# patriciogonzalezvivo/prisma

Measured on AMD Instinct MI355X. Metric: frames/sec (depth_anything ViT-L + flow_raft, 1080p), higher is better.
Workload: dtype split-f16

## Files before the change

include/prisma_bands.h:

```cpp
#ifndef PRISMA_BANDS_H
#define PRISMA_BANDS_H

#include <stddef.h>
#include <stdint.h>

#ifdef __cplusplus
extern "C" {
#endif

typedef struct pb_ctx pb_ctx;

typedef enum {
    PB_OK = 0,
    PB_ERR_ARG = -1,
    PB_ERR_DEVICE = -2,
    PB_ERR_MEMORY = -3,
    PB_ERR_STATE = -4
} pb_status;

typedef enum { PB_F32 = 0, PB_F16 = 1, PB_U8 = 2, PB_I32 = 3 } pb_dtype;

typedef struct {
    const char *name;
    int32_t dtype;
// ... 254 lines not shown
                             void *bits, int inter_rows, float *inter);
int pb_op_mask_matrix_nms(pb_ctx *ctx, const float *inter, const float *area, const int *label, const float *score, int n, float sigma, int guard,
                          float *comp, float *out);
int pb_op_mask_sigmoid_rows(pb_ctx *ctx, const float *logit, int src_rows, int ld, const int *idx, int count, int HW, int guard_rows, float *sig);
int pb_op_mask_dynconv(pb_ctx *ctx, const float *kernels, int src_rows, const int *idx, int row_off, int M, const float *feat, int HW4, int split,
                       int guard_rows, float *out);
int pb_op_mask_band_accumulate(pb_ctx *ctx, const float *sig, const uint8_t *use, int k, int fh, int fw, int h, int w, int H, int W, float thr,
                               int guard, uint8_t *out, uint8_t *inst);
int pb_op_depth_layernorm(pb_ctx *ctx, const float *x, const float *g, const float *b, int B, int ntp, int ntok, int D, int drop_cls, int ldy, int lo_off,
                          int o8_off, float o8_scale, int lo8, int guard_rows, void *out, int *lo8_pa);
int pb_op_depth_attention(pb_ctx *ctx, const float *q, const float *k, const float *v, int B, int heads, int N, int variant, int ldo, int o8_off,
                          float o8_scale, int guard_rows, void *out);
int pb_op_depth_cls_rows(pb_ctx *ctx, const float *cls, const float *pos, int B, int ntp, int D, int guard_rows, float *out);
int pb_op_depth_dpt_tail(pb_ctx *ctx, const float *z, const float *bias, const float *w2, float b2, int B, int H, int W, int OH, int OW, int layout,
                         int ldz, int guard, float *out, int *lo8_pa);
int pb_op_depth_resize_minmax(pb_ctx *ctx, const float *net, int B, int nh, int nw, int H, int W, int guard, float *out, float *mnmx);
int pb_op_zoe_softplus(pb_ctx *ctx, float *x, int rows, int cols, int ld, int guard_rows);
int pb_op_zoe_dot32_relu(pb_ctx *ctx, const float *act, int ld, const float *w2, float b2, int rows, int guard, float *out);
int pb_op_zoe_bilerp_add(pb_ctx *ctx, const float *a, const float *src, int n, int h, int w, int H, int W, int C, int lda, int lds, int ldo,
                         int guard_rows, void *out);
int pb_op_zoe_attractor(pb_ctx *ctx, const float *A, int ldA, int nA, const float *bprev, int n, int h, int w, int H, int W, float alpha,
                        int guard_rows, float *out);
int pb_op_zoe_cat(pb_ctx *ctx, const float *act, int ld_act, const float *rel, const float *emb, int ld_emb, int n, int h, int w, int H, int W,
                  int guard_rows, void *out);
int pb_op_zoe_logbinom_depth(pb_ctx *ctx, const float *pt, int ld_pt, const float *bins, int n, int h, int w, int H, int W, float min_temp,
                             float max_temp, int guard, float *out);
int pb_op_zoe_pil_resize(pb_ctx *ctx, const float *in, int n, int h, int w, int H, int W, int guard, float *out);
int pb_op_bilinear(pb_ctx *ctx, const float *x, float *y, int B, int C, int H, int W, int OH, int OW,
                   int align_corners);
int pb_op_preprocess(pb_ctx *ctx, const uint8_t *frame, int H, int W, float *out, int net_h, int net_w);
// ... 8 lines not shown
```

prisma_amd/_lib.py:

```python
from __future__ import annotations

import ctypes as C
import os

_HERE = os.path.dirname(os.path.abspath(__file__))
LIB_PATH = os.environ.get("PRISMA_BANDS_LIB") or os.path.join(_HERE, "libprisma_bands.so")


class pb_tensor(C.Structure):
    _fields_ = [("name", C.c_char_p), ("dtype", C.c_int32), ("ndim", C.c_int32),
                ("shape", C.c_int64 * 6), ("data", C.c_void_p)]


class pb_depth_cfg(C.Structure):
    _fields_ = [("embed_dim", C.c_int32), ("depth", C.c_int32), ("heads", C.c_int32), ("features", C.c_int32),
                ("out_channels", C.c_int32 * 4), ("pos_grid", C.c_int32), ("max_batch", C.c_int32), ("metric", C.c_int32),
                ("precision", C.c_int32)]


class pb_flow_cfg(C.Structure):
    _fields_ = [("precision", C.c_int32)]


PREC_F16, PREC_SPLIT = 0, 1
# ... 144 lines not shown
    "pb_op_mask_coord_concat": (C.c_int, [_P, _P] + [C.c_int] * 7 + [_P]),
    "pb_op_mask_bilinear": (C.c_int, [_P, _P, _P] + [C.c_int] * 10 + [_P]),
    "pb_op_mask_gn_relu": (C.c_int, [_P, _P, _P, _P] + [C.c_int] * 5 + [_P, _P]),
    "pb_op_mask_cls_points_nms": (C.c_int, [_P, _P] + [C.c_int] * 6 + [_P]),
    "pb_op_mask_gather_rows": (C.c_int, [_P, _P, C.c_int, _P] + [C.c_int] * 5 + [_P]),
    "pb_op_mask_stats": (C.c_int, [_P, _P, C.c_int, C.c_int, C.c_int, C.c_float, C.c_int, _P]),
    "pb_op_mask_intersections": (C.c_int, [_P, _P, C.c_int, C.c_int, _P, C.c_int, C.c_int, C.c_float, C.c_int, _P, C.c_int, _P]),
    "pb_op_mask_matrix_nms": (C.c_int, [_P, _P, _P, _P, _P, C.c_int, C.c_float, C.c_int, _P, _P]),
    "pb_op_mask_sigmoid_rows": (C.c_int, [_P, _P, C.c_int, C.c_int, _P, C.c_int, C.c_int, C.c_int, _P]),
    "pb_op_mask_dynconv": (C.c_int, [_P, _P, C.c_int, _P, C.c_int, C.c_int, _P, C.c_int, C.c_int, C.c_int, _P]),
    "pb_op_mask_band_accumulate": (C.c_int, [_P, _P, _P] + [C.c_int] * 7 + [C.c_float, C.c_int, _P, _P]),
    "pb_op_depth_layernorm": (C.c_int, [_P, _P, _P, _P] + [C.c_int] * 8 + [C.c_float, C.c_int, C.c_int, _P, _P]),
    "pb_op_depth_attention": (C.c_int, [_P, _P, _P, _P] + [C.c_int] * 6 + [C.c_float, C.c_int, _P]),
    "pb_op_depth_cls_rows": (C.c_int, [_P, _P, _P] + [C.c_int] * 4 + [_P]),
    "pb_op_depth_dpt_tail": (C.c_int, [_P, _P, _P, _P, C.c_float] + [C.c_int] * 8 + [_P, _P]),
    "pb_op_depth_resize_minmax": (C.c_int, [_P, _P] + [C.c_int] * 6 + [_P, _P]),
    "pb_op_zoe_softplus": (C.c_int, [_P, _P] + [C.c_int] * 4),
    "pb_op_zoe_dot32_relu": (C.c_int, [_P, _P, C.c_int, _P, C.c_float, C.c_int, C.c_int, _P]),
    "pb_op_zoe_bilerp_add": (C.c_int, [_P, _P, _P] + [C.c_int] * 10 + [_P]),
    "pb_op_zoe_attractor": (C.c_int, [_P, _P, C.c_int, C.c_int, _P] + [C.c_int] * 5 + [C.c_float, C.c_int, _P]),
    "pb_op_zoe_cat": (C.c_int, [_P, _P, C.c_int, _P, _P] + [C.c_int] * 7 + [_P]),
    "pb_op_zoe_logbinom_depth": (C.c_int, [_P, _P, C.c_int, _P] + [C.c_int] * 5 + [C.c_float, C.c_float, C.c_int, _P]),
    "pb_op_zoe_pil_resize": (C.c_int, [_P, _P] + [C.c_int] * 6 + [_P]),
    "pb_op_bilinear": (C.c_int, [_P, _P, _P] + [C.c_int] * 7),
    "pb_op_preprocess": (C.c_int, [_P, _P, C.c_int, C.c_int, _P, C.c_int, C.c_int]),
    "pb_op_encode_depth": (C.c_int, [_P, _P, C.c_int, C.c_int, C.c_int, C.c_int, _P, _P, _P]),
}

_lib = None

# ... 33 lines not shown
```

prisma_amd/csrc/abi_ops.hip:

```cpp
#include <string.h>

#include <algorithm>
#include <vector>

#include "abi_ctx.h"
#include "corr_layout.h"
#include "gmflow_engine.h"
#include "mask_kernels.h"
#include "zoe_kernels.h"

namespace {
enum { SL_F16 = 0, SL_SPLIT16 = 1, SL_MX3 = 2, SL_MX2 = 3 };

class SplitOpEngine : public EngineBase {
  public:
    explicit SplitOpEngine(int device) : EngineBase(device) {}
    int setup(const pb_tensor *t, int n, int layout, int tapin) {
        PB_TRY(begin_load(t, n));
        split_w_ = layout != SL_F16; mx_ = layout >= SL_MX3; pack_mx2_ = layout == SL_MX2; pack_tapin_ = tapin;
        return 0;
    }
    int pack_layer(bool is_conv, int sa, int N, int K, PackedW &w) {
        if (is_conv) return pack_conv("l", true, nullptr, nullptr, w, sa);
        const pb_tensor *tw = find("l.weight"), *tb = find("l.bias");
// ... 831 lines not shown
    int dpt_tail(const float *z, const float *bias, const float *w2, float b2, int B, int H, int W, int OH, int OW, int layout, int ldz, int guard,
                 float *out) {
        const int Zp = 320, lo_off = layout ? Zp : 0;
        const int64_t P = (int64_t)B * H * W, px = (int64_t)B * OH * OW;
        std::vector<float> zp((size_t)P * Zp, 0.f);
        for (int64_t p = 0; p < P; ++p) memcpy(&zp[(size_t)p * Zp], z + p * 288, 288 * 4);
        std::vector<f16> hz((size_t)P * ldz);
        memset(hz.data(), 0xFF, hz.size() * 2);
        build_map(zp.data(), P, Zp, Zp, layout == 0 ? SL_F16 : (layout == 1 ? SL_SPLIT16 : SL_MX3), 1, ldz, hz);
        DevMem dz, dbias, dw2, dout;
        PB_TRY(up(dz, hz.data(), hz.size() * 2)); PB_TRY(up(dbias, bias, 32 * 4)); PB_TRY(up(dw2, w2, 32 * 4));
        PB_TRY(preset(dout, (size_t)(px + guard) * 4));
        PB_TRY(launch_dpt_tail(stream, dz.as<f16>(), B, H, W, ldz, lo_off, layout == 2 ? kLo8Pa : -1, dbias.as<float>(), dw2.as<float>(), b2, dout.as<float>(),
                               OH, OW));
        return finish(out, dout, (size_t)(px + guard) * 4);
    }

    int resize_minmax(const float *net, int B, int nh, int nw, int H, int W, int guard, float *out, float *mnmx) {
        const int64_t px = (int64_t)B * H * W;
        DevMem dn, dout, dmm;
        PB_TRY(up(dn, net, (size_t)B * nh * nw * 4));
        PB_TRY(preset(dout, (size_t)(px + guard) * 4));
        PB_TRY(dmm.alloc((size_t)B * 2 * 4));
        PB_TRY(launch_init_minmax(stream, dmm.as<unsigned>(), B));
        PB_TRY(launch_depth_resize_minmax(stream, dn.as<float>(), B, nh, nw, dout.as<float>(), H, W, dmm.as<unsigned>()));
        PB_TRY(finish(out, dout, (size_t)(px + guard) * 4));
        std::vector<unsigned> mm((size_t)B * 2);
        PB_TRY(down(mm.data(), dmm, mm.size() * 4));
        for (size_t i = 0; i < mm.size(); ++i) {
            const unsigned u = (mm[i] & 0x80000000u) ? (mm[i] & 0x7fffffffu) : ~mm[i];
// ... 1108 lines not shown
    return e.attention(q, k, v, B, heads, N, variant, ldo, o8_off, o8_scale, guard_rows, out);
}
int pb_op_depth_cls_rows(pb_ctx *c, const float *cls, const float *pos, int B, int ntp, int D, int guard_rows, float *out) {
    PB_CHECK(c && cls && pos && out && B > 0 && ntp > 0 && D > 0 && guard_rows >= 0, PB_ERR_ARG, "op_depth_cls_rows: bad arguments");
    DEPTH_OP_ENGINE(e);
    return e.cls_rows(cls, pos, B, ntp, D, guard_rows, out);
}
int pb_op_depth_dpt_tail(pb_ctx *c, const float *z, const float *bias, const float *w2, float b2, int B, int H, int W, int OH, int OW, int layout,
                         int ldz, int guard, float *out, int *lo8_pa) {
    PB_CHECK(c && z && bias && w2 && out && B > 0 && H > 0 && W > 0 && OH > 0 && OW > 0 && layout >= 0 && layout <= 2 && ldz % 8 == 0 &&
                 ldz >= (layout ? 640 : 320) && guard >= 0, PB_ERR_ARG, "op_depth_dpt_tail: bad arguments (a pixel is 320 halfs per part)");
    DEPTH_OP_ENGINE(e);
    if (lo8_pa) *lo8_pa = e.lo8_pa();
    return e.dpt_tail(z, bias, w2, b2, B, H, W, OH, OW, layout, ldz, guard, out);
}
int pb_op_depth_resize_minmax(pb_ctx *c, const float *net, int B, int nh, int nw, int H, int W, int guard, float *out, float *mnmx) {
    PB_CHECK(c && net && out && mnmx && B > 0 && nh > 0 && nw > 0 && H > 0 && W > 0 && guard >= 0, PB_ERR_ARG, "op_depth_resize_minmax: bad arguments");
    DEPTH_OP_ENGINE(e);
    return e.resize_minmax(net, B, nh, nw, H, W, guard, out, mnmx);
}
int pb_op_zoe_softplus(pb_ctx *c, float *x, int rows, int cols, int ld, int guard_rows) {
    PB_CHECK(c && x && rows > 0 && cols > 0 && ld >= cols && guard_rows >= 0, PB_ERR_ARG, "op_zoe_softplus: bad arguments");
    DEPTH_OP_ENGINE(e);
    return e.softplus(x, rows, cols, ld, guard_rows);
}
int pb_op_zoe_dot32_relu(pb_ctx *c, const float *act, int ld, const float *w2, float b2, int rows, int guard, float *out) {
    PB_CHECK(c && act && w2 && out && rows > 0 && ld >= 32 && ld % 8 == 0 && guard >= 0, PB_ERR_ARG, "op_zoe_dot32_relu: bad arguments");
    DEPTH_OP_ENGINE(e);
    return e.dot32_relu(act, ld, w2, b2, rows, guard, out);
}
// ... 35 lines not shown
```

prisma_amd/csrc/elementwise.hip:

```cpp
#include "kernels.h"

namespace {

__global__ __launch_bounds__(256) void layernorm_kernel(const float *__restrict__ x, const float *__restrict__ g,
                                                        const float *__restrict__ bt, f16 *__restrict__ y, int B,
                                                        int ntp, int ntok, int D, float eps, int drop_cls, int ldy,
                                                        int lo_off, int o8_off, float o8_scale, int lo8_pa) {
    const int lane = threadIdx.x & 63;
    const int64_t r = (int64_t)blockIdx.x * 4 + (threadIdx.x >> 6);
    if (r >= (int64_t)B * ntok) return;
    const int b = (int)(r / ntok), t = (int)(r - (int64_t)b * ntok);
    if (drop_cls && t == 0) return;
    const float *xr = x + ((int64_t)b * ntp + t) * D;
    f16 *yr = drop_cls ? y + ((int64_t)b * (ntok - 1) + (t - 1)) * ldy : y + ((int64_t)b * ntp + t) * ldy;
    f32x4 v[4];
    float s = 0.f;
#pragma unroll
    for (int j = 0; j < 4; ++j) {
        const int c = lane * 4 + 256 * j;
        if (c < D) {
            v[j] = *(const f32x4 *)(xr + c);
            s += (v[j][0] + v[j][1]) + (v[j][2] + v[j][3]);
        }
    }
// ... 689 lines not shown
    for (int j = 0; j < 8; ++j) s += fmaxf(acc[j] + bias[q4 * 8 + j], 0.f) * w2[q4 * 8 + j];
    s += __shfl_xor(s, 1);
    s += __shfl_xor(s, 2);
    if (live && q4 == 0) out[((int64_t)b * OH + Y) * OW + X] = fmaxf(s + b2, 0.f);
}

int launch_dpt_tail(hipStream_t s, const f16 *z, int B, int H, int W, int ldz, int lo_off, int lo8_pa, const float *bias, const float *w2, float b2,
                    float *out, int OH, int OW) {
    PB_CHECK(ldz % 8 == 0 && lo_off % 8 == 0 && (int64_t)H * W * ldz * 2 < (1LL << 31), -1, "dpt tail: pixel stride %d / residual offset %d must be multiples of 8, an image below 2 GB", ldz, lo_off);
    const float sy = bilerp_scale(H, OH, 1), sx = bilerp_scale(W, OW, 1);
    hipLaunchKernelGGL(dpt_tail_kernel, dim3((OW + 15) / 16, (OH + 3) / 4, B), dim3(256), 0, s, z, H, W, ldz, lo_off, lo8_pa, sy, sx, bias, w2, b2, out, OH, OW);
    PB_HIP(hipGetLastError());
    return 0;
}

int launch_bilinear_nhwc(hipStream_t s, const f16 *x, f16 *y, int B, int H, int W, int OH, int OW, int C, int ldc,
                         int align, int lo_off, int lo8_pa) {
    PB_CHECK(C % 8 == 0 && ldc % 8 == 0, -1, "bilinear: C=%d ldc=%d must be multiples of 8", C, ldc);
    const float sy = bilerp_scale(H, OH, align), sx = bilerp_scale(W, OW, align);
    hipLaunchKernelGGL(bilinear_nhwc_kernel, dim3(nblk((int64_t)B * OH * OW * (C / 8))), dim3(256), 0, s, x, y, B, H,
                       W, OH, OW, C / 8, ldc, align, sy, sx, lo_off, lo8_pa);
    PB_HIP(hipGetLastError());
    return 0;
}

int launch_init_minmax(hipStream_t s, unsigned *mm, int B) {
    hipLaunchKernelGGL(init_minmax_kernel, dim3(nblk(B)), dim3(256), 0, s, mm, B);
    PB_HIP(hipGetLastError());
    return 0;
}
// ... 95 lines not shown
```

prisma_amd/csrc/engine.h:

```cpp
#pragma once
#include <map>
#include <string>
#include <vector>

#include "engine_base.h"
#include "zoe_kernels.h"

class DepthEngine : public EngineBase {
  public:
    DepthEngine(int device, const pb_depth_cfg &cfg, const CreateEnv &env = create_env());
    int load(const pb_tensor *w, int n);
    int infer(const uint8_t *frames_dev, int n, int H, int W, float *depth_out, uint8_t *rgb_out, float *mn,
              float *mx, int flip);
    int max_batch() const { return cfg_.max_batch > 0 ? cfg_.max_batch : 1; }

  private:
    int prepare(int B, int H, int W);
    int run_chunk(const uint8_t *frames, int n, float *depth_out, uint8_t *rgb_out, float *mn, float *mx, int flip);
    int vit(int n);
    int head(int f0, int n);
    int tail(int n, float *depth_out, uint8_t *rgb_out, float *mn, float *mx, int flip);
    int load_metric();
    int plan_metric(int B, int H, int W);
    int metric_tables(int H, int W);
// ... 9 lines not shown
    int head_tapin_ = 1;
    int vit_sw_ = 0, head_sa_ = 0, head_sw_ = 0, hs_ = 1;
    int vit_res_ = 15;
    int vit_mx_ = 0, head_mx_ = 0;
    int batch_cap(int H, int W) const;
    PackedW patch_;
    float *cls_ = nullptr;
    std::vector<float> pos_host_;
    struct Block { float *ln1g, *ln1b, *ln2g, *ln2b, *ls1, *ls2; PackedW qkv, proj, fc1, fc2; };
    std::vector<Block> blocks_;
    float *normg_ = nullptr, *normb_ = nullptr;
    PackedW proj_[4], rs0_, rs1_, rs3_, rn_[4], outc_[4], rcu_[4][2][2], oc1_, oc2_;
    PackedW wz_;
    int head_tail_ = 1;
    f16 *z_ = nullptr;
    float *w2_ = nullptr;
    float b2_ = 0.f;
    static constexpr int64_t kSkFloats = (int64_t)512 * 128 * 128;

    int pB_ = 0, pH_ = 0, pW_ = 0;
    int hB_ = 1;
    int nh_ = 0, nw_ = 0, gh_ = 0, gw_ = 0, ntok_ = 0, ntp_ = 0, P_ = 0;
    int lh_[4] = {0, 0, 0, 0}, lw_[4] = {0, 0, 0, 0};
    int *xi_ = nullptr, *yi_ = nullptr;
    float *xw_ = nullptr, *yw_ = nullptr, *pos_ = nullptr;
    f16 *patchA_ = nullptr, *Y_ = nullptr, *Q_ = nullptr, *K_ = nullptr, *Vt_ = nullptr, *AO_ = nullptr, *Hd_ = nullptr;
    float *X_ = nullptr;
    f16 *feat_[4] = {nullptr, nullptr, nullptr, nullptr};
    f16 *pj_[4] = {}, *lay_[4] = {}, *rnraw_[4] = {}, *rnrelu_[4] = {}, *tmp_[4] = {}, *sraw_[4] = {}, *srelu_[4] = {},
        *yb_[4] = {}, *ocb_[4] = {}, *path_[4] = {};
// ... 13 lines not shown
```

prisma_amd/csrc/engine.hip:

```cpp
#include "engine.h"

#include <math.h>
#include <stdlib.h>
#include <string.h>

#include <algorithm>

namespace {
const char *const kFam[] = {"gemm_f16", "conv_igemm_f16", "attention", "layernorm", "elementwise", "prepost", "gemm_f16_resid",
                            "gemm_f16_qkv"};
enum { F_GEMM_RESID = 6, F_GEMM_QKV = 7 };
inline int cp64(int c) { return (int)round_up(c, 64); }
}

DepthEngine::DepthEngine(int dev, const pb_depth_cfg &cfg, const CreateEnv &env) : EngineBase(dev, env, kFam), cfg_(cfg) {}

PackSpec DepthEngine::spec(int sa, int sw, int mx2) const {
    PackSpec s;
    s.sa = sa; s.sw = sw; s.mx = head_mx_; s.mx2 = mx2; s.tapin = head_tapin_;
    return s;
}

int DepthEngine::pack_vit(const float *wt, int N, int K, PackedW &out, const float *bias, bool keep_res) {
    if (vit_mx_) return pack_spec(wt, N, K, K, out, bias, 1, keep_res ? spec(0, 1, 1) : spec(0, 0));
// ... 101 lines not shown
        if ((r = pack_conv(Hh + "projects." + std::to_string(i), oc[i], D, 1, true, proj_[i]))) return r;
        if ((r = pack_conv(Hh + "scratch.layer" + std::to_string(i + 1) + "_rn", F, oc[i], 3, false, rn_[i]))) return r;
        const std::string rf = Hh + "scratch.refinenet" + std::to_string(i + 1) + ".";
        if ((r = pack_conv(rf + "out_conv", F, F, 1, true, outc_[i]))) return r;
        for (int u = 0; u < 2; ++u)
            for (int c = 0; c < 2; ++c)
                if ((r = pack_conv(rf + "resConfUnit" + std::to_string(u + 1) + ".conv" + std::to_string(c + 1), F, F, 3,
                                   true, rcu_[i][u][c])))
                    return r;
    }
    if ((r = pack_convT(Hh + "resize_layers.0", oc[0], 4, rs0_))) return r;
    if ((r = pack_convT(Hh + "resize_layers.1", oc[1], 2, rs1_))) return r;
    if ((r = pack_conv(Hh + "resize_layers.3", oc[3], oc[3], 3, true, rs3_))) return r;
    if ((r = pack_conv(Hh + "scratch.output_conv1", F / 2, F, 3, true, oc1_))) return r;
    if ((r = pack_conv(Hh + "scratch.output_conv2.0", 32, F / 2, 3, true, oc2_))) return r;
    head_tail_ = env.head_tail && !cfg_.metric;
    if (head_tail_) {
        const int ci = F / 2, cip = cp64(ci);
        const float *wt = need(Hh + "scratch.output_conv2.0.weight", (int64_t)32 * ci * 9);
        if (!wt) return PB_ERR_ARG;
        std::vector<float> g((size_t)288 * cip, 0.f);
        for (int c = 0; c < 32; ++c)
            for (int k = 0; k < ci; ++k)
                for (int t = 0; t < 9; ++t) g[((size_t)t * 32 + c) * cip + k] = wt[((size_t)c * ci + k) * 9 + t];
        if ((r = pack_spec(g.data(), 288, cip, cip, wz_, nullptr, 1, spec(head_sa_, head_sw_)))) return r;
        wz_.Kreal = ci;
    }
    UP(w2_, Hh + "scratch.output_conv2.2.weight", 32);
    { NEED(b2, Hh + "scratch.output_conv2.2.bias", 1); b2_ = b2[0]; }
#undef NEED
#undef UP
    if (cfg_.metric) {
        int rm = load_metric();
        if (rm) return rm;
    }
    tmap_.clear();
    PB_HIP(hipDeviceSynchronize());
    return 0;
}

namespace {
// ... 129 lines not shown
        const size_t mxs = vit_mx_ ? 3 : 2;
        Y_ = (f16 *)carve((size_t)rows * D * mxs);
        const size_t qkb = (size_t)B * cfg_.heads * ntp_ * 64 * 2 + slack;
        Q_ = (f16 *)carve(qkb); K_ = (f16 *)carve(qkb); Vt_ = (f16 *)carve(qkb);
        AO_ = (f16 *)carve((size_t)rows * D * mxs);
        Hd_ = (f16 *)carve((size_t)rows * 4 * D * mxs);
        for (int i = 0; i < 4; ++i) feat_[i] = (f16 *)carve((size_t)round_up((int64_t)B * P_, 256) * D * 2 * hs_);
        for (int i = 0; i < 4; ++i) {
            const size_t pix = (size_t)round_up((int64_t)HB * lh_[i] * lw_[i], 256) * hs_;
            const int ocp = cp64(cfg_.out_channels[i]);
            pj_[i] = (f16 *)carve((size_t)round_up((int64_t)HB * P_, 256) * ocp * 2 * hs_);
            lay_[i] = i == 2 ? pj_[2] : (f16 *)carve(pix * ocp * 2);
            rnraw_[i] = (f16 *)carve(pix * Fp * 2); rnrelu_[i] = (f16 *)carve(pix * Fp * 2);
            tmp_[i] = (f16 *)carve(pix * Fp * 2);
            sraw_[i] = (f16 *)carve(pix * Fp * 2); srelu_[i] = (f16 *)carve(pix * Fp * 2);
            yb_[i] = (f16 *)carve(pix * Fp * 2); ocb_[i] = (f16 *)carve(pix * Fp * 2);
            const int th = i == 0 ? 2 * lh_[0] : lh_[i - 1], tw = i == 0 ? 2 * lw_[0] : lw_[i - 1];
            path_[i] = (f16 *)carve((size_t)round_up((int64_t)HB * th * tw, 256) * Fp * 2 * hs_);
        }
        o1_ = (f16 *)carve((size_t)round_up((int64_t)HB * 4 * lh_[0] * lw_[0], 256) * F2p * 2 * hs_);
        if (head_tail_) z_ = (f16 *)carve((size_t)round_up((int64_t)HB * 4 * lh_[0] * lw_[0], 256) * cp64(288) * 2 * hs_);
        else up_ = (f16 *)carve((size_t)round_up((int64_t)HB * nh_ * nw_, 256) * F2p * 2 * hs_);
        netd_ = (float *)carve((size_t)HB * nh_ * nw_ * 4);
        full_ = (float *)carve((size_t)HB * H * W * 4);
        mm_ = (unsigned *)carve((size_t)HB * 8);
        return cfg_.metric ? plan_metric(HB, H, W) : 0;
    });
    if (r) return r;
    std::vector<int> xi, yi;
    std::vector<float> xw, yw, pos;
    if (cfg_.metric) {
// ... 142 lines not shown
        if ((r = conv3(lay_[i], cp64(oc[i]), n, lh_[i], lw_[i], rn_[i], rnraw_[i], rnrelu_[i], nullptr, nullptr, ACT_NONE,
                       1, Fp)))
            return r;
        nhwc("layer" + std::to_string(i + 1) + "_rn", rnraw_[i], F, lh_[i], lw_[i], Fp);
    }
    for (int lv = 3; lv >= 0; --lv) {
        const int h = lh_[lv], w = lw_[lv];
        const f16 *sr = rnraw_[lv], *sl = rnrelu_[lv];
        if (lv < 3) {
            if ((r = conv3(rnrelu_[lv], Fp, n, h, w, rcu_[lv][0][0], tmp_[lv], nullptr, nullptr, nullptr, ACT_RELU, 1, Fp))) return r;
            if ((r = conv3(tmp_[lv], Fp, n, h, w, rcu_[lv][0][1], sraw_[lv], srelu_[lv], rnraw_[lv], path_[lv + 1], ACT_NONE, 1, Fp))) return r;
            sr = sraw_[lv]; sl = srelu_[lv];
        }
        if ((r = conv3(sl, Fp, n, h, w, rcu_[lv][1][0], tmp_[lv], nullptr, nullptr, nullptr, ACT_RELU, 1, Fp))) return r;
        if ((r = conv3(tmp_[lv], Fp, n, h, w, rcu_[lv][1][1], yb_[lv], nullptr, sr, nullptr, ACT_NONE, 1, Fp))) return r;
        {
            GemmArgs a;
            a.A = yb_[lv]; a.lda = hs * Fp; a.M = n * h * w; a.out = ocb_[lv]; a.ldo = hs * Fp; a.lo_off = lo(Fp);
            if ((r = gemm(A_DENSE, EPI_STD, a, outc_[lv]))) return r;
        }
        const int th = lv == 0 ? 2 * h : lh_[lv - 1], tw = lv == 0 ? 2 * w : lw_[lv - 1];
        if ((r = bil(ocb_[lv], path_[lv], h, w, th, tw, F, Fp))) return r;
        nhwc("path" + std::to_string(lv + 1), path_[lv], F, th, tw, Fp);
    }
    const int h1 = 2 * lh_[0], w1 = 2 * lw_[0];
    if ((r = conv3(path_[0], Fp, n, h1, w1, oc1_, o1_, nullptr, nullptr, nullptr, ACT_NONE, 1, F2p))) return r;
    nhwc("output_conv1", o1_, F2, h1, w1, F2p);
    if (head_tail_) {
        const int Zp = cp64(288);
        GemmArgs a;
        a.A = o1_; a.lda = hs * F2p; a.M = n * h1 * w1; a.out = z_; a.ldo = hs * Zp; a.lo_off = lo(Zp); a.N = 288;
        if ((r = gemm(A_DENSE, EPI_STD, a, wz_))) return r;
        r = timed(F_ELT, 0, (double)n * ((double)h1 * w1 * 288 * (head_sa_ ? 3.0 : 2.0) + (double)nh_ * nw_ * 4.0), [&] {
            return launch_dpt_tail(stream, z_, n, h1, w1, hs * Zp, lo(Zp), head_mx_ ? kLo8Pa : -1, oc2_.bias, w2_, b2_, netd_, nh_, nw_);
        });
        if (r) return r;
        stages_["net_depth"] = Stage::f32_rows(netd_, n, nh_, nw_);
        return 0;
    }
    if ((r = bil(o1_, up_, h1, w1, nh_, nw_, F2, F2p))) return r;
    if (cfg_.metric) {
// ... 84 lines not shown
```

prisma_amd/csrc/kernels.h:

```cpp
#pragma once
#include "common.h"

int launch_attention(hipStream_t s, const f16 *q, const f16 *k, const f16 *vt, f16 *o, int B, int heads, int ntp,
                     int ntok, int ldo, int variant = 0, int o8_off = 0, float o8_scale = 16.f);

int launch_layernorm(hipStream_t s, const float *x, const float *g, const float *b, f16 *y, int B, int ntp, int ntok,
                     int D, float eps, int drop_cls, int ldy = 0, int lo_off = 0, int o8_off = 0, float o8_scale = 16.f, int lo8_pa = -1);

int launch_cls_rows(hipStream_t s, float *resid, const float *cls, const float *pos, int B, int ntp, int D);

int launch_preprocess(hipStream_t s, const uint8_t *frames, int B, int H, int W, int nh, int nw, const int *xi,
                      const float *xw, const int *yi, const float *yw, f16 *out, int Kp, float *chw_out);

int launch_bilinear_nhwc(hipStream_t s, const f16 *x, f16 *y, int B, int H, int W, int OH, int OW, int C, int ldc,
                         int align_corners, int lo_off = 0, int lo8_pa = -1);

int launch_dpt_tail(hipStream_t s, const f16 *z, int B, int H, int W, int ldz, int lo_off, int lo8_pa, const float *bias, const float *w2, float b2,
                    float *out, int OH, int OW);

int launch_depth_resize_minmax(hipStream_t s, const float *net, int B, int nh, int nw, float *out, int H, int W,
                               unsigned *mm);
int launch_minmax_only(hipStream_t s, const float *x, int B, int64_t per, unsigned *mm);
int launch_heat_encode(hipStream_t s, const float *depth, int B, int H, int W, const unsigned *mm, int flip,
                       uint8_t *rgb, float *mn, float *mx);
int launch_init_minmax(hipStream_t s, unsigned *mm, int B);
int launch_still_encode(hipStream_t s, const float *depth, int H, int W, unsigned *mm, unsigned *g2max, uint8_t *q, int flip, int encode_range,
                        uint8_t *rgb, float *mnmx);
int launch_point_cloud(hipStream_t s, const float *depth, const uint8_t *rgb, int n, int H, int W, int flip, float u0, float v0, float fx,
                       float fy, unsigned *mm, uint8_t *out);
int launch_hue_heat(hipStream_t s, const uint8_t *frames, int n, int H, int W, int y0, int x0, int Hd, int Wd, uint8_t *depth_out, float *heat_out);

int launch_nchw_f32_to_nhwc_f16(hipStream_t s, const float *x, f16 *y, int B, int C, int H, int W, int ldc, int relu);
int launch_nhwc_f16_to_nchw_f32(hipStream_t s, const f16 *x, float *y, int B, int C, int H, int W, int ldc);
// ... 16 lines not shown
```

prisma_amd/engine.py:

```python
from __future__ import annotations

import ctypes as C
from typing import Dict, List, Optional, Tuple

import numpy as np

from . import _lib
from ._lib import check
from .synth import DEPTH_CFGS, MASK_CFGS, DepthCfg, MaskCfg


def _ptr(a: Optional[np.ndarray]):
    return None if a is None else a.ctypes.data_as(C.c_void_p)


def _f32(a) -> np.ndarray:
    return np.ascontiguousarray(a, dtype=np.float32)


VERTEX_DTYPE = np.dtype([("x", "<f4"), ("y", "<f4"), ("z", "<f4"), ("red", "u1"), ("green", "u1"), ("blue", "u1")])


def device_count() -> int:
    return _lib.load().pb_device_count()
# ... 966 lines not shown
    def depth_cls_rows(self, cls, pos, B: int, ntp: int, guard_rows: int = 2) -> np.ndarray:
        cls, pos = _f32(cls), _f32(pos)
        out = np.empty((B * ntp + guard_rows, cls.shape[0]), np.float32)
        check(self.lib.pb_op_depth_cls_rows(self.ctx, _ptr(cls), _ptr(pos), B, ntp, cls.shape[0], guard_rows, _ptr(out)))
        return out

    def depth_dpt_tail(self, z, bias, w2, b2: float, OH: int, OW: int, layout: int, ldz: int, guard: int = 64):
        z, bias, w2 = _f32(z), _f32(bias), _f32(w2)
        B, H, W, Cc = z.shape
        assert Cc == 288 and bias.shape == (32,) and w2.shape == (32,)
        out = np.empty(B * OH * OW + guard, np.float32)
        pa = C.c_int(-1)
        check(self.lib.pb_op_depth_dpt_tail(self.ctx, _ptr(z), _ptr(bias), _ptr(w2), b2, B, H, W, OH, OW, layout, ldz, guard, _ptr(out), C.byref(pa)))
        return out, pa.value

    def depth_resize_minmax(self, net, H: int, W: int, guard: int = 64):
        net = _f32(net)
        B, nh, nw = net.shape
        out = np.empty(B * H * W + guard, np.float32)
        mm = np.empty((B, 2), np.float32)
        check(self.lib.pb_op_depth_resize_minmax(self.ctx, _ptr(net), B, nh, nw, H, W, guard, _ptr(out), _ptr(mm)))
        return out, mm

    def zoe_softplus(self, buf, rows: int, cols: int) -> np.ndarray:
        buf = _f32(buf).copy()
        check(self.lib.pb_op_zoe_softplus(self.ctx, _ptr(buf), rows, cols, buf.shape[1], buf.shape[0] - rows))
        return buf

    def zoe_dot32_relu(self, act, ld: int, w2, b2: float, guard: int = 8) -> np.ndarray:
        act, w2 = _f32(act), _f32(w2)
# ... 351 lines not shown
```

Before: 138.0.

## Fold refinenet1 out_conv into output_conv1 and run conv after upsample as gather

The refinenet1 1x1 out_conv weights are composed with the 3x3 output_conv1 weights on the host at setup. One GEMM now runs at low resolution and produces 9 taps times F/2 channels. A new gather kernel then bilinearly upsamples those per-tap partial sums and adds them at the 2x resolution. This replaces the path of 1x1 conv, bilinear upsample to a full-width buffer, then a 3x3 conv at high resolution, so high-resolution FLOPs and traffic drop. The cost is a wider intermediate (9*F/2 channels) and composed weights whose rounding differs slightly. It is on by default unless the head_tail env bit 2 is set.

```diff
diff --git a/include/prisma_bands.h b/include/prisma_bands.h
--- a/include/prisma_bands.h
+++ b/include/prisma_bands.h
@@ -292,6 +292,8 @@
 int pb_op_depth_cls_rows(pb_ctx *ctx, const float *cls, const float *pos, int B, int ntp, int D, int guard_rows, float *out);
 int pb_op_depth_dpt_tail(pb_ctx *ctx, const float *z, const float *bias, const float *w2, float b2, int B, int H, int W, int OH, int OW, int layout,
                          int ldz, int guard, float *out, int *lo8_pa);
+int pb_op_depth_oc1(pb_ctx *ctx, const float *x, const float *wo, const float *bo, const float *w1, const float *b1, int B, int H, int W, int F, int layout,
+                    int route, int guard_rows, void *out, int *lo8_pa);
 int pb_op_depth_resize_minmax(pb_ctx *ctx, const float *net, int B, int nh, int nw, int H, int W, int guard, float *out, float *mnmx);
 int pb_op_zoe_softplus(pb_ctx *ctx, float *x, int rows, int cols, int ld, int guard_rows);
 int pb_op_zoe_dot32_relu(pb_ctx *ctx, const float *act, int ld, const float *w2, float b2, int rows, int guard, float *out);
diff --git a/prisma_amd/_lib.py b/prisma_amd/_lib.py
--- a/prisma_amd/_lib.py
+++ b/prisma_amd/_lib.py
@@ -182,6 +182,7 @@
     "pb_op_depth_attention": (C.c_int, [_P, _P, _P, _P] + [C.c_int] * 6 + [C.c_float, C.c_int, _P]),
     "pb_op_depth_cls_rows": (C.c_int, [_P, _P, _P] + [C.c_int] * 4 + [_P]),
     "pb_op_depth_dpt_tail": (C.c_int, [_P, _P, _P, _P, C.c_float] + [C.c_int] * 8 + [_P, _P]),
+    "pb_op_depth_oc1": (C.c_int, [_P] * 6 + [C.c_int] * 7 + [_P, _P]),
     "pb_op_depth_resize_minmax": (C.c_int, [_P, _P] + [C.c_int] * 6 + [_P, _P]),
     "pb_op_zoe_softplus": (C.c_int, [_P, _P] + [C.c_int] * 4),
     "pb_op_zoe_dot32_relu": (C.c_int, [_P, _P, C.c_int, _P, C.c_float, C.c_int, C.c_int, _P]),
diff --git a/prisma_amd/csrc/abi_ops.hip b/prisma_amd/csrc/abi_ops.hip
--- a/prisma_amd/csrc/abi_ops.hip
+++ b/prisma_amd/csrc/abi_ops.hip
@@ -6,6 +6,7 @@
 #include "abi_ctx.h"
 #include "corr_layout.h"
 #include "gmflow_engine.h"
+#include "head_linear.h"
 #include "mask_kernels.h"
 #include "zoe_kernels.h"
 
@@ -869,6 +870,37 @@
         PB_TRY(launch_dpt_tail(stream, dz.as<f16>(), B, H, W, ldz, lo_off, layout == 2 ? kLo8Pa : -1, dbias.as<float>(), dw2.as<float>(), b2, dout.as<float>(),
                                OH, OW));
         return finish(out, dout, (size_t)(px + guard) * 4);
+    }
+
+    int oc1(const float *x, const float *wo, const float *bo, const float *w1, const float *b1, int B, int H, int W, int F, int layout, int route, int guard,
+            void *out) {
+        const int F2 = F / 2, F2p = (int)round_up(F2, 64), sa = layout != SL_F16, hs = sa ? 2 : 1, Zp = (int)round_up(9 * F2, 64);
+        const int64_t P = (int64_t)B * H * W, OP = 4 * P, ldo = hs * F2p;
+        const int lo8 = layout == SL_MX3 ? kLo8Pa : -1;
+        std::vector<f16> hx((size_t)round_up(P, 256) * hs * F, (f16)0.f);
+        build_map(x, P, F, F, layout, sa, hs * F, hx);
+        DevMem dx, db1, dout, dz, dp;
+        PB_TRY(up(dx, hx.data(), hx.size() * 2)); PB_TRY(up(db1, b1, (size_t)F2 * 4));
+        PB_TRY(preset(dout, (size_t)(round_up(OP, 256) + guard) * ldo * 2));
+        if (route) {
+            std::vector<double> g, gb;
+            pb_compose_oc1(w1, wo, bo, F, F, g, gb);
+            const std::vector<float> gf(g.begin(), g.end()), gbf(gb.begin(), gb.end());
+            PackedW wz;
+            PB_TRY(pack(gf.data(), 9 * F2, F, F, wz, gbf.data(), 1, sa));
+            PB_TRY(preset(dz, (size_t)round_up(P, 256) * hs * Zp * 2));
+            PB_TRY(dense(dx.as<f16>(), hs * F, P, wz, dz.as<f16>(), hs * Zp, ACT_NONE, nullptr, 0, -1, sa ? Zp : 0));
+            PB_TRY(launch_dpt_oc1_gather(stream, dz.as<f16>(), B, H, W, F2, hs * Zp, sa ? Zp : 0, lo8, db1.as<float>(), dout.as<f16>(), (int)ldo, sa ? F2p : 0));
+        } else {
+            PackedW wc, w3;
+            PB_TRY(pack(wo, F, F, F, wc, bo, 1, sa));
+            PB_TRY(pack(pb_conv_rows(w1, F2, F, 9, F).data(), F2, 9 * F, 9 * F, w3, b1, 9, sa));
+            PB_TRY(preset(dz, (size_t)round_up(P, 256) * hs * F * 2)); PB_TRY(preset(dp, (size_t)round_up(OP, 256) * hs * F * 2));
+            PB_TRY(dense(dx.as<f16>(), hs * F, P, wc, dz.as<f16>(), hs * F, ACT_NONE, nullptr, 0, -1, sa ? F : 0));
+            PB_TRY(launch_bilinear_nhwc(stream, dz.as<f16>(), dp.as<f16>(), B, H, W, 2 * H, 2 * W, F, hs * F, 1, sa ? F : 0, lo8));
+            PB_TRY(conv(dp.as<f16>(), F, 0, B, 2 * H, 2 * W, 3, 3, 1, w3, dout.as<f16>(), (int)ldo, ACT_NONE, 0, nullptr, nullptr, sa ? F2p : 0));
+        }
+        return finish(out, dout, (size_t)(OP + guard) * ldo * 2);
     }
 
     int resize_minmax(const float *net, int B, int nh, int nw, int H, int W, int guard, float *out, float *mnmx) {
@@ -2007,6 +2039,16 @@
     if (lo8_pa) *lo8_pa = e.lo8_pa();
     return e.dpt_tail(z, bias, w2, b2, B, H, W, OH, OW, layout, ldz, guard, out);
 }
+int pb_op_depth_oc1(pb_ctx *c, const float *x, const float *wo, const float *bo, const float *w1, const float *b1, int B, int H, int W, int F, int layout,
+                    int route, int guard_rows, void *out, int *lo8_pa) {
+    PB_CHECK(c && x && wo && bo && w1 && b1 && out && B > 0 && H > 0 && W > 0 && F > 0 && F % 64 == 0 && layout >= SL_F16 && layout <= SL_MX3 &&
+                 (route == 0 || route == 1) && guard_rows >= 0, PB_ERR_ARG, "op_depth_oc1: bad arguments (F a multiple of 64; layout 0 f16, 1 split16, 2 mx3)");
+    PB_HIP(hipSetDevice(c->device));
+    DepthOpEngine e(c->device);
+    PB_TRY(e.setup(nullptr, 0, layout, 1));
+    if (lo8_pa) *lo8_pa = e.lo8_pa();
+    return e.oc1(x, wo, bo, w1, b1, B, H, W, F, layout, route, guard_rows, out);
+}
 int pb_op_depth_resize_minmax(pb_ctx *c, const float *net, int B, int nh, int nw, int H, int W, int guard, float *out, float *mnmx) {
     PB_CHECK(c && net && out && mnmx && B > 0 && nh > 0 && nw > 0 && H > 0 && W > 0 && guard >= 0, PB_ERR_ARG, "op_depth_resize_minmax: bad arguments");
     DEPTH_OP_ENGINE(e);
diff --git a/prisma_amd/csrc/elementwise.hip b/prisma_amd/csrc/elementwise.hip
--- a/prisma_amd/csrc/elementwise.hip
+++ b/prisma_amd/csrc/elementwise.hip
@@ -727,6 +727,117 @@
     return 0;
 }
 
+__global__ __launch_bounds__(256) void dpt_oc1_gather_kernel(const f16 *__restrict__ z, int H, int W, int C, int ldz, int lo_off, int lo8_pa, float sy, float sx,
+                                                             const float *__restrict__ bias, f16 *__restrict__ out, int ldo, int olo_off, int OH, int OW,
+                                                             int TW, int TH) {
+    const int C8 = C >> 3, cg = threadIdx.x % C8, p = threadIdx.x / C8;
+    const int X = blockIdx.x * TW + p % TW, Y = blockIdx.y * TH + p / TW, b = blockIdx.z;
+    if (p >= TW * TH || X >= OW || Y >= OH) return;
+    int y0[3], y1[3], x0[3], x1[3];
+    float ly[3], lx[3];
+    bool oky[3], okx[3];
+#pragma unroll
+    for (int t = 0; t < 3; ++t) {
+        const int qy = Y + t - 1, qx = X + t - 1;
+        oky[t] = qy >= 0 && qy < OH; okx[t] = qx >= 0 && qx < OW;
+        bilerp_src(oky[t] ? qy : 0, sy, H, 1, y0[t], y1[t], ly[t]);
+        bilerp_src(okx[t] ? qx : 0, sx, W, 1, x0[t], x1[t], lx[t]);
+    }
+    const __amdgpu_buffer_rsrc_t rs = make_rsrc(z + (int64_t)b * H * W * ldz, (unsigned)((int64_t)H * W * ldz * 2));
+    const int lane_ch = cg * 8;
+    typedef int i32x4v __attribute__((ext_vector_type(4)));
+    typedef int i32x2v __attribute__((ext_vector_type(2)));
+    const float inv = __builtin_ldexpf(1.f, -(lo8_pa + 12));
+    float acc[8];
+#pragma unroll
+    for (int j = 0; j < 8; ++j) acc[j] = 0.f;
+#pragma unroll
+    for (int ky = 0; ky < 3; ++ky)
+#pragma unroll
+        for (int kx = 0; kx < 3; ++kx) {
+            if (!(oky[ky] && okx[kx])) continue;
+            const int ch = (ky * 3 + kx) * C + lane_ch;
+            const int o[4] = {(y0[ky] * W + x0[kx]) * ldz, (y0[ky] * W + x1[kx]) * ldz, (y1[ky] * W + x0[kx]) * ldz, (y1[ky] * W + x1[kx]) * ldz};
+            const float hy = 1.f - ly[ky], hx = 1.f - lx[kx];
+            const float w4[4] = {hy * hx, hy * lx[kx], ly[ky] * hx, ly[ky] * lx[kx]};
+            f16x8 h[4];
+#pragma unroll
+            for (int n = 0; n < 4; ++n) h[n] = __builtin_bit_cast(f16x8, (i32x4v)__builtin_amdgcn_raw_buffer_load_b128(rs, (o[n] + ch) * 2, 0, 0));
+            if (lo_off && lo8_pa >= 0) {
+                int2 u[4];
+#pragma unroll
+                for (int n = 0; n < 4; ++n) {
+                    const i32x2v t2 = (i32x2v)__builtin_amdgcn_raw_buffer_load_b64(rs, o[n] * 2 + 3 * lo_off + ch, 0, 0);
+                    u[n].x = t2[0]; u[n].y = t2[1];
+                }
+#pragma unroll
+                for (int n = 0; n < 4; ++n) {
+                    const float wl = w4[n] * inv;
+#pragma unroll
+                    for (int j = 0; j < 8; ++j) acc[j] += w4[n] * (float)h[n][j];
+#pragma unroll
+                    for (int hh = 0; hh < 2; ++hh) {
+                        const int wv = hh ? u[n].y : u[n].x;
+                        const f32x2 a = __builtin_amdgcn_cvt_pk_f32_fp8(wv, false), d = __builtin_amdgcn_cvt_pk_f32_fp8(wv, true);
+                        acc[4 * hh + 0] += wl * a[0]; acc[4 * hh + 1] += wl * a[1]; acc[4 * hh + 2] += wl * d[0]; acc[4 * hh + 3] += wl * d[1];
+                    }
+                }
+            } else if (lo_off) {
+#pragma unroll
+                for (int n = 0; n < 4; ++n) {
+                    const f16x8 l = __builtin_bit_cast(f16x8, (i32x4v)__builtin_amdgcn_raw_buffer_load_b128(rs, (o[n] + ch + lo_off) * 2, 0, 0));
+#pragma unroll
+                    for (int j = 0; j < 8; ++j) acc[j] += w4[n] * ((float)h[n][j] + (float)l[j]);
+                }
+            } else {
+#pragma unroll
+                for (int n = 0; n < 4; ++n)
+#pragma unroll
+                    for (int j = 0; j < 8; ++j) acc[j] += w4[n] * (float)h[n][j];
+            }
+        }
+    const float4 b0 = *(const float4 *)(bias + lane_ch), b1 = *(const float4 *)(bias + lane_ch + 4);
+    const float bs[8] = {b0.x, b0.y, b0.z, b0.w, b1.x, b1.y, b1.z, b1.w};
+    f16 *dst = out + (((int64_t)b * OH + Y) * OW + X) * ldo + lane_ch;
+    f16x8 o;
+#pragma unroll
+    for (int j = 0; j < 8; ++j) {
+        acc[j] += bs[j];
+        o[j] = (f16)acc[j];
+    }
+    *(f16x8 *)dst = o;
+    if (olo_off && lo8_pa >= 0) {
+        const float shi = __builtin_ldexpf(1.f, lo8_pa), slo = __builtin_ldexpf(1.f, lo8_pa + 12);
+        int2 h8, l8;
+        h8.x = pb_fp8x4((float)o[0] * shi, (float)o[1] * shi, (float)o[2] * shi, (float)o[3] * shi);
+        h8.y = pb_fp8x4((float)o[4] * shi, (float)o[5] * shi, (float)o[6] * shi, (float)o[7] * shi);
+        l8.x = pb_fp8x4((acc[0] - (float)o[0]) * slo, (acc[1] - (float)o[1]) * slo, (acc[2] - (float)o[2]) * slo, (acc[3] - (float)o[3]) * slo);
+        l8.y = pb_fp8x4((acc[4] - (float)o[4]) * slo, (acc[5] - (float)o[5]) * slo, (acc[6] - (float)o[6]) * slo, (acc[7] - (float)o[7]) * slo);
+        char *d8 = (char *)(dst - lane_ch) + lane_ch;
+        *(int2 *)(d8 + 2 * olo_off) = h8;
+        *(int2 *)(d8 + 3 * olo_off) = l8;
+    } else if (olo_off) {
+        f16x8 l;
+#pragma unroll
+        for (int j = 0; j < 8; ++j) l[j] = (f16)(acc[j] - (float)o[j]);
+        *(f16x8 *)(dst + olo_off) = l;
+    }
+}
+
+int launch_dpt_oc1_gather(hipStream_t s, const f16 *z, int B, int H, int W, int C, int ldz, int lo_off, int lo8_pa, const float *bias, f16 *out, int ldo,
+                          int olo_off) {
+    PB_CHECK(C > 0 && C % 8 == 0 && C <= 2048 && ldz % 8 == 0 && lo_off % 8 == 0 && ldo % 8 == 0 && olo_off % 8 == 0 && !lo_off == !olo_off &&
+                 (int64_t)H * W * ldz * 2 < (1LL << 31), -1,
+             "oc1 gather: %d channels, pixel strides %d / %d, residual offsets %d / %d must be multiples of 8, an image below 2 GB", C, ldz, ldo, lo_off, olo_off);
+    const int OH = 2 * H, OW = 2 * W;
+    const float sy = bilerp_scale(H, OH, 1), sx = bilerp_scale(W, OW, 1);
+    const int PB = 256 / (C / 8), TH = PB >= 16 ? 4 : (PB >= 4 ? 2 : 1), TW = PB / TH;
+    hipLaunchKernelGGL(dpt_oc1_gather_kernel, dim3((OW + TW - 1) / TW, (OH + TH - 1) / TH, B), dim3(256), 0, s, z, H, W, C, ldz, lo_off, lo8_pa, sy, sx, bias, out,
+                       ldo, olo_off, OH, OW, TW, TH);
+    PB_HIP(hipGetLastError());
+    return 0;
+}
+
 int launch_bilinear_nhwc(hipStream_t s, const f16 *x, f16 *y, int B, int H, int W, int OH, int OW, int C, int ldc,
                          int align, int lo_off, int lo8_pa) {
     PB_CHECK(C % 8 == 0 && ldc % 8 == 0, -1, "bilinear: C=%d ldc=%d must be multiples of 8", C, ldc);
diff --git a/prisma_amd/csrc/engine.h b/prisma_amd/csrc/engine.h
--- a/prisma_amd/csrc/engine.h
+++ b/prisma_amd/csrc/engine.h
@@ -47,6 +47,9 @@
     PackedW wz_;
     int head_tail_ = 1;
     f16 *z_ = nullptr;
+    PackedW wo1_;
+    int head_oc1_ = 1;
+    f16 *zo_ = nullptr;
     float *w2_ = nullptr;
     float b2_ = 0.f;
     static constexpr int64_t kSkFloats = (int64_t)512 * 128 * 128;
diff --git a/prisma_amd/csrc/engine.hip b/prisma_amd/csrc/engine.hip
--- a/prisma_amd/csrc/engine.hip
+++ b/prisma_amd/csrc/engine.hip
@@ -5,6 +5,8 @@
 #include <string.h>
 
 #include <algorithm>
+
+#include "head_linear.h"
 
 namespace {
 const char *const kFam[] = {"gemm_f16", "conv_igemm_f16", "attention", "layernorm", "elementwise", "prepost", "gemm_f16_resid",
@@ -139,7 +141,7 @@
     if ((r = pack_conv(Hh + "resize_layers.3", oc[3], oc[3], 3, true, rs3_))) return r;
     if ((r = pack_conv(Hh + "scratch.output_conv1", F / 2, F, 3, true, oc1_))) return r;
     if ((r = pack_conv(Hh + "scratch.output_conv2.0", 32, F / 2, 3, true, oc2_))) return r;
-    head_tail_ = env.head_tail && !cfg_.metric;
+    head_tail_ = (env.head_tail & 1) && !cfg_.metric;
     if (head_tail_) {
         const int ci = F / 2, cip = cp64(ci);
         const float *wt = need(Hh + "scratch.output_conv2.0.weight", (int64_t)32 * ci * 9);
@@ -150,6 +152,18 @@
                 for (int t = 0; t < 9; ++t) g[((size_t)t * 32 + c) * cip + k] = wt[((size_t)c * ci + k) * 9 + t];
         if ((r = pack_spec(g.data(), 288, cip, cip, wz_, nullptr, 1, spec(head_sa_, head_sw_)))) return r;
         wz_.Kreal = ci;
+    }
+    head_oc1_ = !(env.head_tail & 2) && !cfg_.metric;
+    if (head_oc1_) {
+        const std::string oc = Hh + "scratch.refinenet1.out_conv";
+        const float *w1 = need(Hh + "scratch.output_conv1.weight", (int64_t)(F / 2) * F * 9);
+        const float *wo = need(oc + ".weight", (int64_t)F * F), *bo = need(oc + ".bias", F);
+        if (!w1 || !wo || !bo) return PB_ERR_ARG;
+        std::vector<double> g, gb;
+        pb_compose_oc1(w1, wo, bo, F, F, g, gb);
+        const std::vector<float> gf(g.begin(), g.end()), gbf(gb.begin(), gb.end());
+        if ((r = pack_spec(gf.data(), 9 * (F / 2), F, F, wo1_, gbf.data(), 1, spec(head_sa_, head_sw_)))) return r;
+        wo1_.Kreal = F;
     }
     UP(w2_, Hh + "scratch.output_conv2.2.weight", 32);
     { NEED(b2, Hh + "scratch.output_conv2.2.bias", 1); b2_ = b2[0]; }
@@ -309,7 +323,13 @@
             rnraw_[i] = (f16 *)carve(pix * Fp * 2); rnrelu_[i] = (f16 *)carve(pix * Fp * 2);
             tmp_[i] = (f16 *)carve(pix * Fp * 2);
             sraw_[i] = (f16 *)carve(pix * Fp * 2); srelu_[i] = (f16 *)carve(pix * Fp * 2);
-            yb_[i] = (f16 *)carve(pix * Fp * 2); ocb_[i] = (f16 *)carve(pix * Fp * 2);
+            yb_[i] = (f16 *)carve(pix * Fp * 2);
+            if (i == 0 && head_oc1_) {
+                ocb_[0] = path_[0] = nullptr;
+                zo_ = (f16 *)carve(pix * cp64(9 * (F / 2)) * 2);
+                continue;
+            }
+            ocb_[i] = (f16 *)carve(pix * Fp * 2);
             const int th = i == 0 ? 2 * lh_[0] : lh_[i - 1], tw = i == 0 ? 2 * lw_[0] : lw_[i - 1];
             path_[i] = (f16 *)carve((size_t)round_up((int64_t)HB * th * tw, 256) * Fp * 2 * hs_);
         }
@@ -482,6 +502,7 @@
         }
         if ((r = conv3(sl, Fp, n, h, w, rcu_[lv][1][0], tmp_[lv], nullptr, nullptr, nullptr, ACT_RELU, 1, Fp))) return r;
         if ((r = conv3(tmp_[lv], Fp, n, h, w, rcu_[lv][1][1], yb_[lv], nullptr, sr, nullptr, ACT_NONE, 1, Fp))) return r;
+        if (lv == 0 && head_oc1_) break;
         {
             GemmArgs a;
             a.A = yb_[lv]; a.lda = hs * Fp; a.M = n * h * w; a.out = ocb_[lv]; a.ldo = hs * Fp; a.lo_off = lo(Fp);
@@ -492,7 +513,16 @@
         nhwc("path" + std::to_string(lv + 1), path_[lv], F, th, tw, Fp);
     }
     const int h1 = 2 * lh_[0], w1 = 2 * lw_[0];
-    if ((r = conv3(path_[0], Fp, n, h1, w1, oc1_, o1_, nullptr, nullptr, nullptr, ACT_NONE, 1, F2p))) return r;
+    if (head_oc1_) {
+        const int Zp = cp64(9 * F2);
+        GemmArgs a;
+        a.A = yb_[0]; a.lda = hs * Fp; a.M = n * lh_[0] * lw_[0]; a.out = zo_; a.ldo = hs * Zp; a.lo_off = lo(Zp); a.N = 9 * F2;
+        if ((r = gemm(A_DENSE, EPI_STD, a, wo1_))) return r;
+        r = timed(F_ELT, 0, (double)n * ((double)lh_[0] * lw_[0] * 9 * F2 * (head_sa_ ? 3.0 : 2.0) + (double)h1 * w1 * F2 * 2.0 * hs), [&] {
+            return launch_dpt_oc1_gather(stream, zo_, n, lh_[0], lw_[0], F2, hs * Zp, lo(Zp), head_mx_ ? kLo8Pa : -1, oc1_.bias, o1_, hs * F2p, lo(F2p));
+        });
+        if (r) return r;
+    } else if ((r = conv3(path_[0], Fp, n, h1, w1, oc1_, o1_, nullptr, nullptr, nullptr, ACT_NONE, 1, F2p))) return r;
     nhwc("output_conv1", o1_, F2, h1, w1, F2p);
     if (head_tail_) {
         const int Zp = cp64(288);
diff --git a/prisma_amd/csrc/head_linear.h b/prisma_amd/csrc/head_linear.h
--- /dev/null
+++ b/prisma_amd/csrc/head_linear.h
@@ -0,0 +1,22 @@
+#pragma once
+#include <stddef.h>
+
+#include <vector>
+
+template <class T>
+inline void pb_compose_oc1(const T *W1, const T *Wo, const T *bo, int F, int ldk, std::vector<double> &g, std::vector<double> &gb) {
+    const int F2 = F / 2;
+    g.assign((size_t)9 * F2 * ldk, 0.0);
+    gb.assign((size_t)9 * F2, 0.0);
+    for (int t = 0; t < 9; ++t)
+        for (int c = 0; c < F2; ++c) {
+            double *row = g.data() + ((size_t)t * F2 + c) * ldk, b = 0.0;
+            for (int m = 0; m < F; ++m) {
+                const double w = (double)W1[((size_t)c * F + m) * 9 + t];
+                const T *wo = Wo + (size_t)m * F;
+                for (int k = 0; k < F; ++k) row[k] += w * (double)wo[k];
+                b += w * (double)bo[m];
+            }
+            gb[(size_t)t * F2 + c] = b;
+        }
+}
diff --git a/prisma_amd/csrc/kernels.h b/prisma_amd/csrc/kernels.h
--- a/prisma_amd/csrc/kernels.h
+++ b/prisma_amd/csrc/kernels.h
@@ -17,6 +17,9 @@
 
 int launch_dpt_tail(hipStream_t s, const f16 *z, int B, int H, int W, int ldz, int lo_off, int lo8_pa, const float *bias, const float *w2, float b2,
                     float *out, int OH, int OW);
+
+int launch_dpt_oc1_gather(hipStream_t s, const f16 *z, int B, int H, int W, int C, int ldz, int lo_off, int lo8_pa, const float *bias, f16 *out, int ldo,
+                          int olo_off);
 
 int launch_depth_resize_minmax(hipStream_t s, const float *net, int B, int nh, int nw, float *out, int H, int W,
                                unsigned *mm);
diff --git a/prisma_amd/engine.py b/prisma_amd/engine.py
--- a/prisma_amd/engine.py
+++ b/prisma_amd/engine.py
@@ -1004,6 +1004,16 @@
         check(self.lib.pb_op_depth_dpt_tail(self.ctx, _ptr(z), _ptr(bias), _ptr(w2), b2, B, H, W, OH, OW, layout, ldz, guard, _ptr(out), C.byref(pa)))
         return out, pa.value
 
+    def depth_oc1(self, x, wo, bo, w1, b1, layout: int, route: int = 1, guard_rows: int = 8):
+        x, wo, bo, w1, b1 = _f32(x), _f32(wo), _f32(bo), _f32(w1), _f32(b1)
+        B, H, W, F = x.shape
+        assert wo.shape == (F, F) and bo.shape == (F,) and w1.shape == (F // 2, F, 3, 3) and b1.shape == (F // 2,)
+        F2p = -(-(F // 2) // 64) * 64
+        out = np.empty((B * 4 * H * W + guard_rows, 2 * F2p * (2 if layout else 1)), np.uint8)
+        pa = C.c_int(-1)
+        check(self.lib.pb_op_depth_oc1(self.ctx, _ptr(x), _ptr(wo), _ptr(bo), _ptr(w1), _ptr(b1), B, H, W, F, layout, route, guard_rows, _ptr(out), C.byref(pa)))
+        return out, pa.value
+
     def depth_resize_minmax(self, net, H: int, W: int, guard: int = 64):
         net = _f32(net)
         B, nh, nw = net.shape
```

New measurement: 139.0, median of 6. No clear change (+0.7%).
